# gabrielmittag/NISQA

Measured on AMD Instinct MI355X. Metric: clips/sec (10 s, 48 kHz), higher is better.
Workload: dtype bf16x6 (every GEMM -- CNN, projection, self-attention, pooling: fp32 operands as three exact bf16 terms, 6 MFMA products per term pair, f32 accumulate: all 24 operand mantissa bits; mel f32)

## Files before the change

nisqa_amd/csrc/cnn_bf16.hip:

```cpp
#include "common.hpp"
#include "layout.hpp"
#include <stdlib.h>
#include <atomic>
#include "conv_bf16.hpp"
#include "internal.hpp"
#include "../../include/nisqa_hip.h"
#define NQ_RING2 3
#define NQ_RING34 3

#define FB_RS1 48
#define FB_P1 (168 * FB_RS1)
#define FB_RS2 80
#define FB_P2 (60 * FB_RS2)
#define FB_RS3 144
#define FB_P3 (60 * FB_RS3)
#define FB_PS (72 * FB_RS3)
#define FB_PATCH(T) ((T) * FB_P1)
#define FB_PPLANE 1700
#define FB_ZADDR 2048u
#define FB_BASE 2176u
#define FB_WAVE(T) (((T) * (FB_P1 + FB_PPLANE) + 63u) / 64u * 64u)
#define FB_WGS(T) ((T) == 2 ? 2 : 1)
#define FB_LDS(T) (FB_BASE + 4 * FB_WAVE(T))
static_assert(FB_WAVE(2) == 19584 && FB_LDS(2) == 80512 && 2 * FB_LDS(2) <= 160 * 1024, "two terms: two workgroups (8 waves) per CU");
static_assert(FB_WAVE(3) == 29312 && FB_LDS(3) == 119424 && FB_LDS(3) <= 160 * 1024 && 2 * FB_LDS(3) > 160 * 1024, "three terms: one workgroup per CU");
#define FB_PLAN_OK(T) (FB_PATCH(T) + (T) * FB_PPLANE <= FB_WAVE(T) && (T) * FB_P3 <= FB_WAVE(T) && (T) * FB_PS <= 2 * FB_WAVE(T))
static_assert(FB_PLAN_OK(2) && FB_PLAN_OK(3), "LDS plan");

__device__ constexpr int bwin75_lo(int b) { return b == 0 ? 0 : b == 1 ? 1 : b == 2 ? 2 : b == 3 ? 4 : 5; }
__device__ constexpr int bwin75_hi(int b) { return b == 0 ? 2 : b == 1 ? 3 : b == 2 ? 5 : b == 3 ? 6 : 7; }
__device__ constexpr int bwin53_lo(int b) { return b == 0 ? 0 : b == 1 ? 1 : 3; }
__device__ constexpr int bwin53_hi(int b) { return b == 0 ? 2 : b == 1 ? 4 : 5; }

NQ_CLK_EXPORT(g_phase_clk, nisqa_debug_phase_clock)
NQ_CLK_EXPORT(g_phase_clk6, nisqa_debug_phase_clock6)

#define FB_TAB5 0u
#define FB_TAB6 1024u
NQ_DEV f32x2_t lds_ld64(unsigned a) { return *(NQ_AS3 const f32x2_t*)(a); }
template <int FMT>
NQ_DEV float epi_fmt(float v, float c, float t) {
    return FMT == NQ_FMT_BF16X3 || FMT == NQ_FMT_BF16X6 ? fmaxf(v + t, 0.f) : fmaxf(fmaf(v, c, t), 0.f);
}

template <int FMT, int CIN, int MT, int NT, int W, int RS, int PLANE, bool APF, int RING>
NQ_DEV void fb_conv_k(f32x16 (&acc)[MT][NT], __amdgpu_buffer_rsrc_t wrs, int wbyte, unsigned lane16, const unsigned (&base)[MT],
                      const unsigned (&m9)[MT], conv_k_ring<FMT == NQ_FMT_BF16X6 ? 3 : 2, NT, 3>& ring) {
    if constexpr (FMT == NQ_FMT_BF16X6) conv_k_terms_ring<3, CIN, MT, NT, W, RS, PLANE, FB_ZADDR, 3, true, true>(acc, wrs, wbyte, lane16, base, m9, ring);
    else conv_k_bf16<CIN, MT, NT, W, RS, PLANE, FB_ZADDR, APF, RING, FMT>(acc, wrs, wbyte, lane16, base, m9);
}

template <int FMT, bool SEGX, bool P3>
NQ_DEV void cnn_front_split_body(
    const float* __restrict__ mel_tm, const int32_t* __restrict__ frame_off,
    const int32_t* __restrict__ tok_off, const int32_t* __restrict__ n_wins,
    const float* __restrict__ clip_floor, int n_clips, int seg_hop,
    const float* __restrict__ cw, const unsigned short* __restrict__ wb, float* __restrict__ p3,
    float* __restrict__ feat, const float* __restrict__ seg_x, int seg_L,
    const uint32_t* __restrict__ clip_max_enc, float top_db) {
    extern __shared__ __attribute__((aligned(16))) char smem[];
    constexpr bool X6 = FMT == NQ_FMT_BF16X6, F16 = FMT == NQ_FMT_F16X3 || FMT == NQ_FMT_F16X4;
    constexpr int T = X6 ? 3 : 2;
    static_assert(!P3 || FMT == NQ_FMT_BF16X3, "the fp32 copy of the pooled conv4 tensor is a bf16x3 debug output");
    constexpr int W1_ = X6 ? CNNX_W1 : CNNB_W1, W2_ = X6 ? CNNX_W2 : CNNB_W2, W3_ = X6 ? CNNX_W3 : CNNB_W3, W4_ = X6 ? CNNX_W4 : CNNB_W4,
                  W5_ = X6 ? CNNX_W5 : CNNB_W5, W6_ = X6 ? CNNX_W6 : CNNB_W6, WU16_ = X6 ? CNNX_U16S : CNNB_U16S;
    const int* __restrict__ meta_i = (const int*)(wb + CNNH_META);
    const float* __restrict__ meta_f = (const float*)(wb + CNNH_META);
    float dummy_mx = 0.f;
    NQ_STAMP_BEGIN();
    const int lane = threadIdx.x & 63;
    const int wave = __builtin_amdgcn_readfirstlane(threadIdx.x >> 6);
    const int p0 = blockIdx.x * 4;
    const int b = __builtin_amdgcn_readfirstlane(find_segment_wave(tok_off, n_clips, p0, lane));
    const int k0 = p0 - tok_off[b];
    const int nvalid = min(4, n_wins[b] - k0);
    if (nvalid <= 0) return;
    const bool valid = wave < nvalid;
    const int p = p0 + wave, k = k0 + wave;
    const unsigned R = FB_BASE + wave * FB_WAVE(T);
    const unsigned lane16 = lane * 16;
// ... 10 lines not shown
        vraw[q] = (valid && (q < 11 || lane < 16)) ? src[i0] : 0.f;
    }
    const float tn1 = cw[CNN_T1 + (lane & 15)], tn2 = cw[CNN_T2 + (lane & 31)];
    const float tn3[2] = {cw[CNN_T3 + (lane & 31)], cw[CNN_T3 + 32 + (lane & 31)]};
    const float tn4[2] = {cw[CNN_T4 + (lane & 31)], cw[CNN_T4 + 32 + (lane & 31)]};
    const float tn5 = cw[CNN_T5 + 16 * wave + (lane & 15)], tn6 = cw[CNN_T6 + 16 * wave + (lane & 15)];
    float vin[12];
#pragma unroll
    for (int q = 0; q < 12; ++q) vin[q] = !valid ? 0.f : SEGX ? vraw[q] : fmaxf(vraw[q], fl);
    int e_in = 0;
    float m_in = 0.f;
    float s0 = 1.f;
    if (F16) {
        float mr = 0.f;
#pragma unroll
        for (int q = 0; q < 12; ++q) mr = fmaxf(mr, __builtin_fabsf(vin[q]));
        m_in = wave_max_nonneg(mr);
        e_in = f16_scale_exp(m_in);
        s0 = pow2_f32(e_in);
    }
    {
        const unsigned pb = R + FB_PATCH(T);
        constexpr int NZ = (T * FB_PPLANE + 15) / 16;
#pragma unroll
        for (int it = 0; it < (NZ + 63) / 64; ++it)
            if (64 * it + 64 <= NZ || lane < NZ - 64 * it) lds_st128(pb + (lane + 64 * it) * 16, f32x4{0.f, 0.f, 0.f, 0.f});
        if (lane < 32) ((unsigned*)(smem + FB_ZADDR))[lane] = 0u;
        __builtin_amdgcn_wave_barrier();
        if (!SEGX) {
            unsigned ob[3];
#pragma unroll
            for (int u = 0; u < 3; ++u) {
                const int e = lane + 16 * u, j0 = e >= 48 ? 1 : 0, m = e - 48 * j0;
                ob[u] = pb + ((j0 + 1) * 50 + m + 1) * 2;
            }
#pragma unroll
            for (int q = 0; q < 12; q += 2) {
                const float v0 = vin[q] * s0, v1 = vin[q + 1] * s0;
                lds_store_pair_fmt<FMT>(ob[q % 3] + (q + q / 3) * 100, ob[(q + 1) % 3] + (q + 1 + (q + 1) / 3) * 100, FB_PPLANE, v0, v1,
                                               dummy_mx, true, q + 1 < 11 || lane < 16);
            }
        } else {
#pragma unroll
            for (int q = 0; q < 12; ++q) {
                const int i0 = lane + 64 * q;
                const int m = i0 / 15, j = i0 - 15 * m;
                if (i0 < 720) lds_store_one_fmt<FMT>(pb + ((j + 1) * 50 + (m + 1)) * 2, FB_PPLANE, vin[q] * s0, dummy_mx);
            }
        }
    }
    __builtin_amdgcn_wave_barrier();
    NQ_STAMP(1);

    const int i = lane & 31, hfi = (i >> 2) & 1, qi = (i & 3) + 4 * (i >> 3);
    const int n = lane & 31, hf = lane >> 5, h = lane >> 5;

    conv_k_ring<T, 1, 3> ring2;
    if constexpr (X6) conv_k_preload(ring2, wrs, W2_ * 2, lane16);
    {
        f32x4 w1[1][T];
#pragma unroll
        for (int t = 0; t < T; ++t) w1[0][t] = wfrag_load(wrs, lane16, (W1_ + t * 512) * 2);
        float tn = tn1, c1 = 1.f, ms1 = 0.f;
        int e1 = 0;
        if (F16) {
            e1 = f16_scale_exp(fmaf(m_in, meta_f[8], meta_f[16]));
            c1 = pow2_f32(e1 - e_in - meta_i[0]);
            tn = tn1 * pow2_f32(e1);
        }
        const int xq = min(qi, 14);
        unsigned rd_a = R + FB_PATCH(T) + ((xq + (h ? 2 : 0)) * 50 + 24 * hfi) * 2;
        unsigned rd_b = R + FB_PATCH(T) + ((xq + (h ? 2 : 1)) * 50 + 24 * hfi) * 2;
        const bool is_b = (n & 16) != 0;
        const unsigned mb = is_b ? ~0u : 0u;
        unsigned wr = R + (12 * hf * 7) * FB_RS1 + (n & 15) * 2 + (is_b ? FB_RS1 : 0);
        for (int g2 = 0; g2 < 6; ++g2) {
            f32x16 acc[2][1];
            f32x4 xa[2][T];
#pragma unroll
            for (int tt = 0; tt < 2; ++tt)
#pragma unroll
                for (int t = 0; t < T; ++t) {
                    const unsigned pa = rd_a + 4 * tt + t * FB_PPLANE, pq = rd_b + 4 * tt + t * FB_PPLANE;
                    xa[tt][t] = f32x4{__uint_as_float(lds_ld32(pa)), __uint_as_float(lds_ld32(pa + 4)),
                                      __uint_as_float(lds_ld32(pq)), __uint_as_float(lds_ld32(pq + 4))};
                }
            acc[0][0] = zero16();
            acc[1][0] = zero16();
            if constexpr (X6) {
                mma_terms<T, 2, 1>(acc, xa, w1);
            } else {
                const f32x4 (&w)[T] = w1[0];
                if (FMT == NQ_FMT_F16X4) { acc[0][0] = mfma32_fmt<FMT>(xa[0][1], w[1], acc[0][0]); acc[1][0] = mfma32_fmt<FMT>(xa[1][1], w[1], acc[1][0]); }
                acc[0][0] = mfma32_fmt<FMT>(xa[0][1], w[0], acc[0][0]); acc[1][0] = mfma32_fmt<FMT>(xa[1][1], w[0], acc[1][0]);
                acc[0][0] = mfma32_fmt<FMT>(xa[0][0], w[1], acc[0][0]); acc[1][0] = mfma32_fmt<FMT>(xa[1][0], w[1], acc[1][0]);
                acc[0][0] = mfma32_fmt<FMT>(xa[0][0], w[0], acc[0][0]); acc[1][0] = mfma32_fmt<FMT>(xa[1][0], w[0], acc[1][0]);
            }
            unsigned r[14];
#pragma unroll
            for (int v = 0; v < 14; ++v) {
                const int tt = v / 7, bb = v - 7 * tt;
                const float mx = fmaxf(fmaxf(acc[tt][0][2 * bb], acc[tt][0][2 * bb + 1]), acc[tt][0][2 * bb + 2]);
                r[v] = __float_as_uint(epi_fmt<FMT>(mx, c1, tn));
            }
            unsigned got[7];
#pragma unroll
            for (int kk = 0; kk < 7; ++kk)
                got[kk] = (unsigned)__builtin_amdgcn_ds_swizzle((int)((r[2 * kk] & mb) | (r[2 * kk + 1] & ~mb)), 0x401F);
            float fin[7];
#pragma unroll
            for (int kk = 0; kk < 7; ++kk) {
                const unsigned own = (r[2 * kk + 1] & mb) | (r[2 * kk] & ~mb);
                fin[kk] = __uint_as_float(max(own, got[kk]));
            }
#pragma unroll
            for (int kk = 0; kk < 6; kk += 2) lds_store_pair_fmt<FMT>(wr + 2 * kk * FB_RS1, wr + 2 * (kk + 1) * FB_RS1, FB_P1, fin[kk], fin[kk + 1], ms1);
            lds_store_one_fmt<FMT>(wr + 12 * FB_RS1, FB_P1, fin[6], ms1);
            rd_a += 8; rd_b += 8;
            wr += 14 * FB_RS1;
        }
        if (F16) { m_in = wave_max_nonneg(ms1) * pow2_f32(-e1); e_in = e1; }
    }

    NQ_STAMP(2);
    conv_k_ring<T, 2, 3> ring34;
    {
        f32x16 acc[6][1];
        unsigned base[6], m9[6];
#pragma unroll
        for (int t = 0; t < 6; ++t) {
            acc[t][0] = zero16();
            const int u = 16 * t + qi;
            const int gl = u / 14, w = u % 14, yy = w / 7;
            const int py = 2 * (6 * hfi + gl) + yy, px = w - 7 * yy;
            m9[t] = tap_mask(u < 84, py, px, 24, 7);
            base[t] = R + ((py - 1) * 7 + (px - 1)) * FB_RS1 + (h << 4);
        }
        fb_conv_k<FMT, 16, 6, 1, 7, FB_RS1, FB_P1, false, NQ_RING2>(acc, wrs, W2_ * 2, lane16, base, m9, ring2);
        NQ_STAMP(3);
        if constexpr (X6) {
            conv_k_preload(ring34, wrs, W3_ * 2, lane16);
            __builtin_amdgcn_sched_barrier(0);
        }
        float tn = tn2, c2 = 1.f, ms2 = 0.f;
        int e2 = 0;
        if (F16) {
            e2 = f16_scale_exp(fmaf(m_in, meta_f[9], meta_f[17]));
            c2 = pow2_f32(e2 - e_in - meta_i[1]);
            tn = tn2 * pow2_f32(e2);
        }
        const unsigned wr = R + (6 * hf * 5) * FB_RS2 + n * 2;
#pragma unroll
        for (int k2 = 0; k2 < 30; k2 += 2) {
            float pv[2];
#pragma unroll
            for (int e = 0; e < 2; ++e) {
                const int gl = (k2 + e) / 5, bb = (k2 + e) % 5;
                float mx = -3.0e38f;
#pragma unroll
                for (int yy = 0; yy < 2; ++yy)
#pragma unroll
                    for (int x = bwin75_lo(bb); x < bwin75_hi(bb); ++x) {
                        const int u = 14 * gl + 7 * yy + x;
                        mx = fmaxf(mx, acc[u >> 4][0][u & 15]);
                    }
                pv[e] = epi_fmt<FMT>(mx, c2, tn);
            }
            lds_store_pair_fmt<FMT>(wr + k2 * FB_RS2, wr + (k2 + 1) * FB_RS2, FB_P2, pv[0], pv[1], ms2);
        }
        if (F16) { m_in = wave_max_nonneg(ms2) * pow2_f32(-e2); e_in = e2; }
    }

    NQ_STAMP(4);
    unsigned base34[2], m34[2];
#pragma unroll
    for (int t = 0; t < 2; ++t) {
        const int u = 16 * t + qi;
        const int gl = u / 10, w = u % 10, yy = w / 5;
        const int py = 2 * (3 * hfi + gl) + yy, px = w - 5 * yy;
        m34[t] = tap_mask(u < 30, py, px, 12, 5);
        base34[t] = (py - 1) * 5 + (px - 1);
    }

    {
        f32x16 acc[2][2];
        unsigned base[2];
#pragma unroll
        for (int t = 0; t < 2; ++t) {
#pragma unroll
            for (int nt = 0; nt < 2; ++nt) acc[t][nt] = zero16();
            base[t] = R + base34[t] * FB_RS2 + (h << 4);
        }
        fb_conv_k<FMT, 32, 2, 2, 5, FB_RS2, FB_P2, true, NQ_RING34>(acc, wrs, W3_ * 2, lane16, base, m34, ring34);
        NQ_STAMP(5);
        if constexpr (X6) {
            conv_k_preload(ring34, wrs, W4_ * 2, lane16);
            __builtin_amdgcn_sched_barrier(0);
        }
        float tn[2] = {tn3[0], tn3[1]}, c3 = 1.f, ms3 = 0.f;
        int e3 = 0;
        if (F16) {
            e3 = f16_scale_exp(fmaf(m_in, meta_f[10], meta_f[18]));
            c3 = pow2_f32(e3 - e_in - meta_i[2]);
            tn[0] *= pow2_f32(e3);
            tn[1] *= pow2_f32(e3);
        }
        const unsigned wr = R + (6 * hf * 5) * FB_RS3 + n * 2;
#pragma unroll
        for (int nt = 0; nt < 2; ++nt)
#pragma unroll
            for (int t = 0; t < 2; ++t)
#pragma unroll
                for (int r = 0; r < 16; r += 2) {
                    const int u = 16 * t + r;
                    if (u < 30)
                        lds_store_pair_fmt<FMT>(wr + u * FB_RS3 + 64 * nt, wr + (u + 1) * FB_RS3 + 64 * nt, FB_P3,
                                                epi_fmt<FMT>(acc[t][nt][r], c3, tn[nt]), epi_fmt<FMT>(acc[t][nt][r + 1], c3, tn[nt]), ms3);
                }
        if (F16) { m_in = wave_max_nonneg(ms3) * pow2_f32(-e3); e_in = e3; }
    }

    NQ_STAMP(6);
    const unsigned S4 = FB_BASE;
    const unsigned S5 = FB_BASE + 2 * FB_WAVE(T);
    const int w5b = __builtin_amdgcn_readfirstlane((W5_ + wave * (18 * T * 512)) * 2);
    const int w6b = __builtin_amdgcn_readfirstlane((W6_ + wave * (18 * T * 512)) * 2);
    f32x4 b5[4][T], b6[8][T];
    {
        f32x16 acc[2][2];
        unsigned base[2];
#pragma unroll
        for (int t = 0; t < 2; ++t) {
#pragma unroll
            for (int nt = 0; nt < 2; ++nt) acc[t][nt] = zero16();
            base[t] = R + base34[t] * FB_RS3 + (h << 4);
        }
        fb_conv_k<FMT, 64, 2, 2, 5, FB_RS3, FB_P3, true, NQ_RING34>(acc, wrs, W4_ * 2, lane16, base, m34, ring34);
        NQ_STAMP(7);
        float tn[2] = {tn4[0], tn4[1]}, c4 = 1.f, ms4 = 0.f;
        int e4 = 0;
        if (F16) {
            e4 = f16_scale_exp(fmaf(m_in, meta_f[11], meta_f[19]));
            c4 = pow2_f32(e4 - e_in - meta_i[3]);
            tn[0] *= pow2_f32(e4);
            tn[1] *= pow2_f32(e4);
        }
#pragma unroll
        for (int g = 0; g < 3; ++g)
#pragma unroll
            for (int q = 0; q < T; ++q) b5[g][q] = wfrag_load(wrs, lane16, w5b + (g * T + q) * 1024);
        __syncthreads();
        const unsigned wr = S4 + (18 * wave + 9 * hf) * FB_RS3 + n * 2;
        float* dst = P3 ? p3 + (size_t)p * (18 * 64) : nullptr;
#pragma unroll
        for (int gl = 0; gl < 3; ++gl)
#pragma unroll
            for (int bb = 0; bb < 3; ++bb) {
                float pv[2];
#pragma unroll
                for (int nt = 0; nt < 2; ++nt) {
                    float mx = -3.0e38f;
#pragma unroll
                    for (int yy = 0; yy < 2; ++yy)
#pragma unroll
                        for (int x = bwin53_lo(bb); x < bwin53_hi(bb); ++x) {
                            const int u = 10 * gl + 5 * yy + x;
                            mx = fmaxf(mx, acc[u >> 4][nt][u & 15]);
                        }
                    pv[nt] = epi_fmt<FMT>(mx, c4, tn[nt]);
                    if (P3 && valid) dst[((3 * hf + gl) * 3 + bb) * 64 + n + 32 * nt] = pv[nt];
                }
                lds_store_pair_fmt<FMT>(wr + (gl * 3 + bb) * FB_RS3, wr + (gl * 3 + bb) * FB_RS3 + 64, FB_PS, pv[0], pv[1], ms4);
            }
        if (F16) {
            const float m4 = wave_max_nonneg(ms4) * pow2_f32(-e4);
            const int e5 = f16_scale_exp(fmaf(m4, meta_f[12], meta_f[20]));
            if (lane < 18) {
                lds_st32(FB_TAB5 + (18 * wave + lane) * 8, __float_as_uint(pow2_f32(e5 - e4 - meta_i[4])));
                lds_st32(FB_TAB5 + (18 * wave + lane) * 8 + 4, __float_as_uint(pow2_f32(e5)));
            }
            if (lane < 6) lds_st32(FB_TAB6 + (6 * wave + lane) * 4, __float_as_uint(pow2_f32(-(e5 + meta_i[5]))));
        }
    }
    __syncthreads();
    NQ_STAMP(8);

    {
        const int i16 = lane & 15, kg = lane >> 4;
        const int ch = 16 * wave + i16;
        f32x4 acc5[5];
        unsigned base5[5], m5[5];
#pragma unroll
        for (int t = 0; t < 5; ++t) {
            acc5[t] = f32x4{0.f, 0.f, 0.f, 0.f};
            const int rho = 16 * t + i16;
            const int slot = rho / 18, pix = rho - 18 * slot, ry = pix / 3, rx = pix - 3 * ry;
            m5[t] = tap_mask(rho < 72, ry, rx, 6, 3);
            base5[t] = S4 + (slot * 18 + (ry - 1) * 3 + (rx - 1)) * FB_RS3 + (kg << 4);
        }
        unsigned a5ad[5][T];
        f32x4 a5[2][5][T];
        auto load_a5 = [&](int g) {
            const int tap = g >> 1, s = g & 1;
            const int tapoff = ((tap / 3) * 3 + tap % 3) * FB_RS3;
            if (s == 0) {
#pragma unroll
                for (int t = 0; t < 5; ++t) {
                    const bool ok = (m5[t] >> tap) & 1u;
#pragma unroll
                    for (int q = 0; q < T; ++q) a5ad[t][q] = ok ? base5[t] + q * FB_PS : FB_ZADDR - tapoff;
                }
            }
#pragma unroll
            for (int t = 0; t < 5; ++t)
#pragma unroll
                for (int q = 0; q < T; ++q) a5[g & 1][t][q] = lds_ld128(a5ad[t][q] + tapoff + 64 * s);
        };
        load_a5(0);
#pragma unroll
        for (int g = 0; g < 18; ++g) {
            if (g + 3 < 18) {
#pragma unroll
                for (int q = 0; q < T; ++q) b5[(g + 3) & 3][q] = wfrag_load(wrs, lane16, w5b + ((g + 3) * T + q) * 1024);
            }
            if (g + 1 < 18) load_a5(g + 1);
            if constexpr (X6) {
                __builtin_amdgcn_sched_barrier(0);
                mma16_terms<T, 5>(acc5, a5[g & 1], b5[g & 3]);
            } else mma16_pair_fmt<FMT, 5>(acc5, a5[g & 1], b5[g & 3]);
        }
        NQ_STAMP(9);
#pragma unroll
        for (int g = 0; g < 7; ++g)
#pragma unroll
            for (int q = 0; q < T; ++q) b6[g][q] = wfrag_load(wrs, lane16, w6b + (g * T + q) * 1024);
        {
            const unsigned wr = S5 + (4 * kg) * FB_RS3 + ch * 2;
#pragma unroll
            for (int t = 0; t < 5; ++t)
#pragma unroll
                for (int r = 0; r < 4; r += 2)
                    if (t < 4 || kg < 2) {
                        f32x2_t cs0 = {1.f, 1.f}, cs1 = {1.f, 1.f};
                        if (F16) { cs0 = lds_ld64(FB_TAB5 + (16 * t + r) * 8 + kg * 32); cs1 = lds_ld64(FB_TAB5 + (16 * t + r + 1) * 8 + kg * 32); }
                        lds_store_pair_fmt<FMT>(wr + (16 * t + r) * FB_RS3, wr + (16 * t + r + 1) * FB_RS3, FB_PS,
                                                epi_fmt<FMT>(acc5[t][r], cs0[0], tn5 * cs0[1]), epi_fmt<FMT>(acc5[t][r + 1], cs1[0], tn5 * cs1[1]), dummy_mx);
                    }
        }
        __syncthreads();
        NQ_STAMP(10);

        f32x4 acc6[2], acc6b[2];
        unsigned base6[2], m6[2];
#pragma unroll
        for (int t = 0; t < 2; ++t) {
            acc6[t] = f32x4{0.f, 0.f, 0.f, 0.f};
            acc6b[t] = acc6[t];
            const int rho = 16 * t + i16;
            const int slot = rho / 6, y = rho - 6 * slot;
            m6[t] = tap_mask(rho < 24, y, 1, 6, 3);
            base6[t] = S5 + (slot * 18 + (y - 1) * 3) * FB_RS3 + (kg << 4);
        }
        unsigned a6ad[2][T];
        f32x4 a6[2][2][T];
        auto load_a6 = [&](int g) {
            const int tap = g >> 1, s = g & 1;
            const int tapoff = ((tap / 3) * 3 + tap % 3) * FB_RS3;
            if (s == 0) {
#pragma unroll
                for (int t = 0; t < 2; ++t) {
                    const bool ok = (m6[t] >> tap) & 1u;
#pragma unroll
                    for (int q = 0; q < T; ++q) a6ad[t][q] = ok ? base6[t] + q * FB_PS : FB_ZADDR - tapoff;
                }
            }
#pragma unroll
            for (int t = 0; t < 2; ++t)
#pragma unroll
                for (int q = 0; q < T; ++q) a6[g & 1][t][q] = lds_ld128(a6ad[t][q] + tapoff + 64 * s);
        };
        load_a6(0);
#pragma unroll
        for (int g = 0; g < 18; ++g) {
            if (g + 7 < 18) {
#pragma unroll
                for (int q = 0; q < T; ++q) b6[(g + 7) & 7][q] = wfrag_load(wrs, lane16, w6b + ((g + 7) * T + q) * 1024);
            }
            if (g + 1 < 18) load_a6(g + 1);
            f32x4 (&acc)[2] = (g & 1) ? acc6b : acc6;
            if constexpr (X6) {
                __builtin_amdgcn_sched_barrier(0);
                mma16_terms<T, 2>(acc, a6[g & 1], b6[g & 7]);
            } else mma16_pair_fmt<FMT, 2>(acc, a6[g & 1], b6[g & 7]);
        }
        NQ_STAMP(11);
        const unsigned fo = S4 + wave * 2048;
#pragma unroll
        for (int t = 0; t < 2; ++t)
#pragma unroll
            for (int r = 0; r < 4; ++r) {
                const int rho = 16 * t + 4 * kg + r;
                const int slot = rho / 6, y = rho - 6 * slot;
                if (rho < 24) {
                    const float c6 = F16 ? __uint_as_float(lds_ld32(FB_TAB6 + (16 * t + r) * 4 + kg * 16)) : 1.f;
                    lds_st32(fo + (slot * 96 + i16 * 6 + y) * 4, __float_as_uint(epi_fmt<FMT>(acc6[t][r] + acc6b[t][r], c6, tn6)));
                }
            }
        __builtin_amdgcn_wave_barrier();
#pragma unroll
        for (int q0 = 0; q0 < 96; q0 += 64) {
            const int q = q0 + lane;
            const int slot = q / 24;
            if (q < 96 && slot < nvalid)
                *(f32x4*)(feat + (size_t)(p0 + slot) * 384 + 96 * wave + 4 * (q - 24 * slot)) = lds_ld128(fo + 16 * q);
        }
    }
    NQ_STAMP_END((X6 ? g_phase_clk6 : g_phase_clk), ((blockIdx.y * gridDim.x + blockIdx.x) << 2) + wave);
}

#define FB_PARAMS                                                                                                              \
    const float* __restrict__ mel_tm, const int32_t* __restrict__ frame_off, const int32_t* __restrict__ tok_off,             \
    const int32_t* __restrict__ n_wins, const float* __restrict__ clip_floor, int n_clips, int seg_hop,                       \
    const float* __restrict__ cw, const unsigned short* __restrict__ wb, float* __restrict__ p3, float* __restrict__ feat,    \
    const float* __restrict__ seg_x, int seg_L, const uint32_t* __restrict__ clip_max_enc, float top_db
#define FB_ARGS mel_tm, frame_off, tok_off, n_wins, clip_floor, n_clips, seg_hop, cw, wb, p3, feat, seg_x, seg_L, clip_max_enc, top_db
template <bool SEGX, bool P3>
__global__ __launch_bounds__(256, FB_WGS(2)) void cnn_front_bf16_kernel(FB_PARAMS) {
    cnn_front_split_body<NQ_FMT_BF16X3, SEGX, P3>(FB_ARGS);
}
template <bool P4, bool SEGX>
__global__ __launch_bounds__(256, FB_WGS(2)) void cnn_front_f16_kernel(FB_PARAMS) {
    cnn_front_split_body<P4 ? NQ_FMT_F16X4 : NQ_FMT_F16X3, SEGX, false>(FB_ARGS);
}
template <bool SEGX>
__global__ __launch_bounds__(256, FB_WGS(3)) void cnn_front_bf16x6_kernel(FB_PARAMS) {
    cnn_front_split_body<NQ_FMT_BF16X6, SEGX, false>(FB_ARGS);
}

typedef void (*fb_kernel_t)(const float*, const int32_t*, const int32_t*, const int32_t*, const float*, int, int, const float*,
                            const unsigned short*, float*, float*, const float*, int, const uint32_t*, float);
static int fb_launch(int fmt, bool segx, bool p3, const float* mel_tm, const int32_t* frame_off, const int32_t* tok_off,
                     const int32_t* n_wins, const float* clip_floor, const uint32_t* clip_max_enc, float top_db, int32_t n_clips,
                     int32_t total_tok_padded, int32_t seg_hop, const float* cnn_w, const uint16_t* cnn_wb, float* p3_opt, float* feat,
                     const float* seg_x, int32_t seg_L, void* stream) {
    if (n_clips <= 0 || total_tok_padded <= 0 || (total_tok_padded & 31) || seg_hop <= 0 || !cnn_wb || !feat || fmt < 0 || fmt > 3 ||
        (p3 && fmt != 0) || (segx && (!seg_x || seg_L <= 0)) || (!segx && !clip_floor && !clip_max_enc))
// ... 84 lines not shown
```

nisqa_amd/csrc/conv_bf16.hpp:

```cpp
#pragma once
#include "bf16_terms.hpp"

#define NQ_FMT_BF16X3 0
#define NQ_FMT_F16X3 1
#define NQ_FMT_F16X4 2
#define NQ_FMT_BF16X6 3
typedef _Float16 f16x8 __attribute__((ext_vector_type(8)));
typedef _Float16 f16x2_t __attribute__((ext_vector_type(2)));
template <int FMT>
NQ_DEV f32x16 mfma32_fmt(f32x4 a, f32x4 b, f32x16 c) {
    if (FMT == NQ_FMT_BF16X3) return mfma_bf(a, b, c);
    return __builtin_amdgcn_mfma_f32_32x32x16_f16(__builtin_bit_cast(f16x8, a), __builtin_bit_cast(f16x8, b), c, 0, 0, 0);
}
template <int FMT>
NQ_DEV f32x4 mfma16_fmt(f32x4 a, f32x4 b, f32x4 c) {
    if (FMT == NQ_FMT_BF16X3) return mfma_bf16x16(a, b, c);
    return __builtin_amdgcn_mfma_f32_16x16x32_f16(__builtin_bit_cast(f16x8, a), __builtin_bit_cast(f16x8, b), c, 0, 0, 0);
}
template <int FMT, int MT, int NT>
NQ_DEV void mma_pair_fmt(f32x16 (&acc)[MT][NT], const f32x4 (&ah)[MT], const f32x4 (&al)[MT], const f32x4 (&bh)[NT], const f32x4 (&bl)[NT]) {
    if (FMT == NQ_FMT_F16X4) {
#pragma unroll
        for (int t = 0; t < MT; ++t)
#pragma unroll
            for (int nt = 0; nt < NT; ++nt) acc[t][nt] = mfma32_fmt<FMT>(al[t], bl[nt], acc[t][nt]);
    }
#pragma unroll
    for (int t = 0; t < MT; ++t)
#pragma unroll
        for (int nt = 0; nt < NT; ++nt) acc[t][nt] = mfma32_fmt<FMT>(ah[t], bl[nt], acc[t][nt]);
#pragma unroll
    for (int t = 0; t < MT; ++t)
#pragma unroll
        for (int nt = 0; nt < NT; ++nt) acc[t][nt] = mfma32_fmt<FMT>(al[t], bh[nt], acc[t][nt]);
#pragma unroll
    for (int t = 0; t < MT; ++t)
#pragma unroll
        for (int nt = 0; nt < NT; ++nt) acc[t][nt] = mfma32_fmt<FMT>(ah[t], bh[nt], acc[t][nt]);
}
template <int FMT, int MT>
NQ_DEV void mma16_pair_fmt(f32x4 (&acc)[MT], const f32x4 (&a)[MT][2], const f32x4 (&b)[2]) {
    if (FMT == NQ_FMT_F16X4) {
#pragma unroll
        for (int t = 0; t < MT; ++t) acc[t] = mfma16_fmt<FMT>(a[t][1], b[1], acc[t]);
    }
#pragma unroll
    for (int t = 0; t < MT; ++t) acc[t] = mfma16_fmt<FMT>(a[t][0], b[1], acc[t]);
#pragma unroll
    for (int t = 0; t < MT; ++t) acc[t] = mfma16_fmt<FMT>(a[t][1], b[0], acc[t]);
#pragma unroll
    for (int t = 0; t < MT; ++t) acc[t] = mfma16_fmt<FMT>(a[t][0], b[0], acc[t]);
}
NQ_DEV int f16_scale_exp(float bound) {
    const int be = (int)((__float_as_uint(bound) >> 23) & 0xffu);
// ... 61 lines not shown
    if (FMT == NQ_FMT_BF16X3) { lds_store_split2(a0, a1, plane, v0, v1, st0, st1); return; }
    if (FMT == NQ_FMT_BF16X6) { lds_store_terms2<3>(a0, a1, plane, v0, v1, st0, st1); return; }
    const unsigned hi2 = cvt_pk_f16(v0, v1);
    const f32x2_t vv = {v0, v1};
    const f32x2_t hf = __builtin_convertvector(__builtin_bit_cast(f16x2_t, hi2), f32x2_t);
    const f32x2_t r = vv - hf;
    const unsigned lo2 = cvt_pk_f16(r[0], r[1]);
    mx = fmaxf(fmaxf(mx, __builtin_fabsf(v0)), __builtin_fabsf(v1));
    if (st0) { lds_st16(a0, hi2); lds_st16(a0 + plane, lo2); }
    if (st1) { lds_st16_hi(a1, hi2); lds_st16_hi(a1 + plane, lo2); }
}
template <int FMT>
NQ_DEV void lds_store_one_fmt(unsigned a, int plane, float v, float& mx) {
    if (FMT == NQ_FMT_BF16X3) { lds_store_split(a, plane, v); return; }
    if (FMT == NQ_FMT_BF16X6) { lds_store_terms<3>(a, plane, v); return; }
    const unsigned hi = cvt_pk_f16(v, 0.f);
    const float hf = (float)__builtin_bit_cast(f16x2_t, hi)[0];
    const unsigned lo = cvt_pk_f16(v - hf, 0.f);
    mx = fmaxf(mx, __builtin_fabsf(v));
    lds_st16(a, hi);
    lds_st16(a + plane, lo);
}
NQ_DEV f32x16 splat16(float v) { f32x16 r; for (int q = 0; q < 16; ++q) r[q] = v; return r; }
typedef int nq_i32x4 __attribute__((ext_vector_type(4)));
NQ_DEV f32x4 wfrag_load(__amdgpu_buffer_rsrc_t rsrc, unsigned lane16, int byte_off) {
    return __builtin_bit_cast(f32x4, __builtin_amdgcn_raw_buffer_load_b128(rsrc, lane16, byte_off, 0));
}
NQ_DEV unsigned tap_mask(bool valid, int y, int x, int H, int W) {
    unsigned m = 0;
#pragma unroll
    for (int tap = 0; tap < 9; ++tap) {
        const int yy = y + tap / 3 - 1, xx = x + tap % 3 - 1;
        m |= (valid && (unsigned)yy < (unsigned)H && (unsigned)xx < (unsigned)W) ? (1u << tap) : 0u;
    }
    return m;
}

template <int CIN, int MT, int NT, int W, int RS, int PLANE, unsigned ZADDR, bool APF, int RING = 3, int FMT = NQ_FMT_BF16X3>
NQ_DEV void conv_k_bf16(f32x16 (&acc)[MT][NT], __amdgpu_buffer_rsrc_t rsrc, int wbyte, unsigned lane16,
                        const unsigned (&base)[MT], const unsigned (&m9)[MT]) {
    constexpr int S16 = CIN / 16, TOTAL = 9 * S16, AB = APF ? 2 : 1;
    static_assert(ZADDR >= (2 * W + 2) * RS + 32 * S16, "zero block must sit above the largest tap offset");
    f32x4 bh[RING][NT], bl[RING][NT], ah[AB][MT], al[AB][MT];
    unsigned a_hi[MT], a_lo[MT];
    auto load_b = [&](int g, int slot) {
#pragma unroll
        for (int nt = 0; nt < NT; ++nt) {
            bh[slot][nt] = wfrag_load(rsrc, lane16, wbyte + ((g * NT + nt) * 2 + 0) * 1024);
            bl[slot][nt] = wfrag_load(rsrc, lane16, wbyte + ((g * NT + nt) * 2 + 1) * 1024);
        }
    };
    auto load_a = [&](int g, int slot) {
        const int tap = g / S16, s = g - tap * S16;
        const int tapoff = ((tap / 3) * W + tap % 3) * RS;
        if (s == 0) {
#pragma unroll
            for (int t = 0; t < MT; ++t) {
                const bool ok = (m9[t] >> tap) & 1u;
                a_hi[t] = ok ? base[t] : ZADDR - tapoff;
                a_lo[t] = ok ? base[t] + PLANE : ZADDR - tapoff;
            }
        }
#pragma unroll
        for (int t = 0; t < MT; ++t) {
            ah[slot][t] = lds_ld128(a_hi[t] + tapoff + 32 * s);
            al[slot][t] = lds_ld128(a_lo[t] + tapoff + 32 * s);
        }
    };
#pragma unroll
    for (int g = 0; g < RING - 1; ++g) load_b(g, g);
    if (APF) load_a(0, 0);
#pragma unroll
    for (int g = 0; g < TOTAL; ++g) {
        NQ_STEP_FENCE();
        if (g + RING - 1 < TOTAL) load_b(g + RING - 1, (g + RING - 1) % RING);
        if (APF) { if (g + 1 < TOTAL) load_a(g + 1, (g + 1) & 1); } else load_a(g, 0);
        NQ_ISSUE_FENCE();
        const int sa = APF ? (g & 1) : 0, sb = g % RING;
        mma_pair_fmt<FMT, MT, NT>(acc, ah[sa], al[sa], bh[sb], bl[sb]);
    }
}


template <int T>
NQ_DEV void lds_store_terms2(unsigned a0, unsigned a1, int plane, float v0, float v1, bool st0, bool st1) {
    f32x2_t r = {v0, v1};
#pragma unroll
    for (int t = 0; t < T; ++t) {
        const unsigned pk = cvt_pk_bf16(r[0], r[1]);
        if (st0) lds_st16(a0 + t * plane, pk);
        if (st1) lds_st16_hi(a1 + t * plane, pk);
        if (t + 1 < T) {
            const f32x2_t part = {__uint_as_float(pk << 16), __uint_as_float(pk & 0xffff0000u)};
            r = r - part;
        }
    }
}
template <int T>
NQ_DEV void lds_store_terms(unsigned a, int plane, float v) {
    float r = v;
#pragma unroll
    for (int t = 0; t < T; ++t) {
        const unsigned pk = cvt_pk_bf16(r, 0.f);
        lds_st16(a + t * plane, pk);
        if (t + 1 < T) r -= __uint_as_float(pk << 16);
    }
}
template <int T, int NT, int RING = 3>
struct conv_k_ring { f32x4 b[RING][NT][T]; };
template <int T, int NT, int RING>
NQ_DEV void conv_k_preload(conv_k_ring<T, NT, RING>& r, __amdgpu_buffer_rsrc_t rsrc, int wbyte, unsigned lane16) {
#pragma unroll
    for (int g = 0; g < RING - 1; ++g)
#pragma unroll
        for (int nt = 0; nt < NT; ++nt)
#pragma unroll
            for (int t = 0; t < T; ++t) r.b[g][nt][t] = wfrag_load(rsrc, lane16, wbyte + ((g * NT + nt) * T + t) * 1024);
}
template <int T, int CIN, int MT, int NT, int W, int RS, int PLANE, unsigned ZADDR, int RING, bool FENCE, bool PRE>
NQ_DEV void conv_k_terms_ring(f32x16 (&acc)[MT][NT], __amdgpu_buffer_rsrc_t rsrc, int wbyte, unsigned lane16,
                              const unsigned (&base)[MT], const unsigned (&m9)[MT], conv_k_ring<T, NT, RING>& ring) {
    constexpr int S16 = CIN / 16, TOTAL = 9 * S16;
    static_assert(ZADDR >= (2 * W + 2) * RS + 32 * S16, "zero block must sit above the largest tap offset");
    f32x4 a[2][MT][T];
    unsigned a_ad[MT][T];
    auto load_b = [&](int g, int slot) {
#pragma unroll
        for (int nt = 0; nt < NT; ++nt)
#pragma unroll
            for (int t = 0; t < T; ++t) ring.b[slot][nt][t] = wfrag_load(rsrc, lane16, wbyte + ((g * NT + nt) * T + t) * 1024);
    };
    auto load_a = [&](int g, int slot) {
        const int tap = g / S16, s = g - tap * S16;
        const int tapoff = ((tap / 3) * W + tap % 3) * RS;
        if (s == 0) {
#pragma unroll
            for (int m = 0; m < MT; ++m) {
                const bool ok = (m9[m] >> tap) & 1u;
#pragma unroll
                for (int t = 0; t < T; ++t) a_ad[m][t] = ok ? base[m] + t * PLANE : ZADDR - tapoff;
            }
        }
#pragma unroll
        for (int m = 0; m < MT; ++m)
#pragma unroll
            for (int t = 0; t < T; ++t) a[slot][m][t] = lds_ld128(a_ad[m][t] + tapoff + 32 * s);
    };
    if (!PRE) {
#pragma unroll
        for (int g = 0; g < RING - 1; ++g) load_b(g, g);
    }
    load_a(0, 0);
#pragma unroll
    for (int g = 0; g < TOTAL; ++g) {
        if (g + RING - 1 < TOTAL) load_b(g + RING - 1, (g + RING - 1) % RING);
        if (g + 1 < TOTAL) load_a(g + 1, (g + 1) & 1);
        if (FENCE) __builtin_amdgcn_sched_barrier(0);
        mma_terms<T, MT, NT>(acc, a[g & 1], ring.b[g % RING]);
    }
}
template <int T, int CIN, int MT, int NT, int W, int RS, int PLANE, unsigned ZADDR, int RING = 3, bool FENCE = true>
NQ_DEV void conv_k_terms(f32x16 (&acc)[MT][NT], __amdgpu_buffer_rsrc_t rsrc, int wbyte, unsigned lane16,
                         const unsigned (&base)[MT], const unsigned (&m9)[MT]) {
    conv_k_ring<T, NT, RING> ring;
    conv_k_terms_ring<T, CIN, MT, NT, W, RS, PLANE, ZADDR, RING, FENCE, false>(acc, rsrc, wbyte, lane16, base, m9, ring);
}
```

Measured before the change: 63200.

## Pad conv5/conv6 LDS rows, add per-lane zero window, and triple-buffer A loads

Widens the row stride of the conv4-output and conv5-output staging from 144 to 160 bytes, with compile-time checks that every lane group of the conv5/conv6 A-operand 128-bit LDS reads hits distinct bank slots. Out-of-image taps now read from a zeroed window that keeps each lane's bank offset, instead of one shared zero address. The window is cleared in a new per-wave store. In the six-product path, conv5/conv6 A loads become triple-buffered, and explicit sched_group_barrier sequences interleave the LDS reads, global weight loads and MFMAs. The cost is more registers and somewhat more LDS.

```diff
diff --git a/nisqa_amd/csrc/cnn_bf16.hip b/nisqa_amd/csrc/cnn_bf16.hip
--- a/nisqa_amd/csrc/cnn_bf16.hip
+++ b/nisqa_amd/csrc/cnn_bf16.hip
@@ -3,18 +3,20 @@
 #include <stdlib.h>
 #include <atomic>
 #include "conv_bf16.hpp"
+#include "lds_banks.hpp"
 #include "internal.hpp"
 #include "../../include/nisqa_hip.h"
 #define NQ_RING2 3
 #define NQ_RING34 3
 
-#define FB_RS1 48
+#define FB_RS1 nq_lds::RS_A1
 #define FB_P1 (168 * FB_RS1)
-#define FB_RS2 80
+#define FB_RS2 nq_lds::RS_A2
 #define FB_P2 (60 * FB_RS2)
-#define FB_RS3 144
+#define FB_RS3 nq_lds::RS_A3
 #define FB_P3 (60 * FB_RS3)
-#define FB_PS (72 * FB_RS3)
+#define FB_RSS nq_lds::RS_S
+#define FB_PS (72 * FB_RSS)
 #define FB_PATCH(T) ((T) * FB_P1)
 #define FB_PPLANE 1700
 #define FB_ZADDR 2048u
@@ -26,6 +28,13 @@
 static_assert(FB_WAVE(3) == 29312 && FB_LDS(3) == 119424 && FB_LDS(3) <= 160 * 1024 && 2 * FB_LDS(3) > 160 * 1024, "three terms: one workgroup per CU");
 #define FB_PLAN_OK(T) (FB_PATCH(T) + (T) * FB_PPLANE <= FB_WAVE(T) && (T) * FB_P3 <= FB_WAVE(T) && (T) * FB_PS <= 2 * FB_WAVE(T))
 static_assert(FB_PLAN_OK(2) && FB_PLAN_OK(3), "LDS plan");
+#define FB_ZW(T) ((FB_BASE + (T) * FB_PS + 255u) / 256u * 256u)
+#define FB_ZWN (256 + (2 * 3 + 2) * FB_RSS + 64 + 16)
+static_assert(FB_RSS % 16 == 0 && FB_RSS >= 128 && FB_PS % 256 == 0, "S4 / S5 rows; term planes congruent modulo the bank window");
+static_assert(FB_ZW(2) + 4 * 26 * 16 <= FB_BASE + 2 * FB_WAVE(2) && FB_ZW(3) + 4 * 26 * 16 <= FB_BASE + 2 * FB_WAVE(3), "zero window inside the wave 0 / 1 regions, below S5");
+static_assert(4 * 2048 <= 2 * FB_PS, "the feature staging of conv6's epilogue (2 KB per wave) fits S4");
+static_assert(nq_lds::layer_ways<5>(FB_RSS) == 1 && nq_lds::layer_ways<6>(FB_RSS) == 1,
+              "conv5 / conv6: every lane group of every A-operand ds_read_b128 hits 16 distinct slots, out-of-image taps included");
 
 __device__ constexpr int bwin75_lo(int b) { return b == 0 ? 0 : b == 1 ? 1 : b == 2 ? 2 : b == 3 ? 4 : 5; }
 __device__ constexpr int bwin75_hi(int b) { return b == 0 ? 2 : b == 1 ? 3 : b == 2 ? 5 : b == 3 ? 6 : 7; }
@@ -142,7 +151,7 @@
     __builtin_amdgcn_wave_barrier();
     NQ_STAMP(1);
 
-    const int i = lane & 31, hfi = (i >> 2) & 1, qi = (i & 3) + 4 * (i >> 3);
+    const int hfi = nq_lds::row_hfi(lane), qi = nq_lds::row_qi(lane);
     const int n = lane & 31, hf = lane >> 5, h = lane >> 5;
 
     conv_k_ring<T, 1, 3> ring2;
@@ -220,11 +229,9 @@
 #pragma unroll
         for (int t = 0; t < 6; ++t) {
             acc[t][0] = zero16();
-            const int u = 16 * t + qi;
-            const int gl = u / 14, w = u % 14, yy = w / 7;
-            const int py = 2 * (6 * hfi + gl) + yy, px = w - 7 * yy;
-            m9[t] = tap_mask(u < 84, py, px, 24, 7);
-            base[t] = R + ((py - 1) * 7 + (px - 1)) * FB_RS1 + (h << 4);
+            const nq_lds::pixel px = nq_lds::conv2_pixel(t, qi, hfi);
+            m9[t] = tap_mask(px.valid, px.y, px.x, 24, 7);
+            base[t] = R + nq_lds::a32_base(px, 7, FB_RS1, h);
         }
         fb_conv_k<FMT, 16, 6, 1, 7, FB_RS1, FB_P1, false, NQ_RING2>(acc, wrs, W2_ * 2, lane16, base, m9, ring2);
         NQ_STAMP(3);
@@ -265,11 +272,9 @@
     unsigned base34[2], m34[2];
 #pragma unroll
     for (int t = 0; t < 2; ++t) {
-        const int u = 16 * t + qi;
-        const int gl = u / 10, w = u % 10, yy = w / 5;
-        const int py = 2 * (3 * hfi + gl) + yy, px = w - 5 * yy;
-        m34[t] = tap_mask(u < 30, py, px, 12, 5);
-        base34[t] = (py - 1) * 5 + (px - 1);
+        const nq_lds::pixel px = nq_lds::conv34_pixel(t, qi, hfi);
+        m34[t] = tap_mask(px.valid, px.y, px.x, 12, 5);
+        base34[t] = nq_lds::a32_base(px, 5, 1, 0);
     }
 
     {
@@ -340,7 +345,9 @@
 #pragma unroll
             for (int q = 0; q < T; ++q) b5[g][q] = wfrag_load(wrs, lane16, w5b + (g * T + q) * 1024);
         __syncthreads();
-        const unsigned wr = S4 + (18 * wave + 9 * hf) * FB_RS3 + n * 2;
+        static_assert(4 * 26 * 16 >= FB_ZWN, "zero window: one 16-byte store of 26 lanes per wave");
+        if (lane < 26) lds_st128(FB_ZW(T) + (26 * wave + lane) * 16, f32x4{0.f, 0.f, 0.f, 0.f});
+        const unsigned wr = S4 + (18 * wave + 9 * hf) * FB_RSS + n * 2;
         float* dst = P3 ? p3 + (size_t)p * (18 * 64) : nullptr;
 #pragma unroll
         for (int gl = 0; gl < 3; ++gl)
@@ -360,7 +367,7 @@
                     pv[nt] = epi_fmt<FMT>(mx, c4, tn[nt]);
                     if (P3 && valid) dst[((3 * hf + gl) * 3 + bb) * 64 + n + 32 * nt] = pv[nt];
                 }
-                lds_store_pair_fmt<FMT>(wr + (gl * 3 + bb) * FB_RS3, wr + (gl * 3 + bb) * FB_RS3 + 64, FB_PS, pv[0], pv[1], ms4);
+                lds_store_pair_fmt<FMT>(wr + (gl * 3 + bb) * FB_RSS, wr + (gl * 3 + bb) * FB_RSS + 64, FB_PS, pv[0], pv[1], ms4);
             }
         if (F16) {
             const float m4 = wave_max_nonneg(ms4) * pow2_f32(-e4);
@@ -379,45 +386,55 @@
         const int i16 = lane & 15, kg = lane >> 4;
         const int ch = 16 * wave + i16;
         f32x4 acc5[5];
-        unsigned base5[5], m5[5];
+        unsigned base5[5], zb5[5], m5[5];
 #pragma unroll
         for (int t = 0; t < 5; ++t) {
             acc5[t] = f32x4{0.f, 0.f, 0.f, 0.f};
-            const int rho = 16 * t + i16;
-            const int slot = rho / 18, pix = rho - 18 * slot, ry = pix / 3, rx = pix - 3 * ry;
-            m5[t] = tap_mask(rho < 72, ry, rx, 6, 3);
-            base5[t] = S4 + (slot * 18 + (ry - 1) * 3 + (rx - 1)) * FB_RS3 + (kg << 4);
+            const nq_lds::pixel px = nq_lds::conv5_pixel(t, i16);
+            m5[t] = tap_mask(px.valid, px.y, px.x, 6, 3);
+            base5[t] = S4 + nq_lds::a16_base(nq_lds::conv5_slot(t, i16), px, FB_RSS, kg);
+            zb5[t] = nq_lds::zero_window_base(FB_ZW(T), base5[t]);
         }
         unsigned a5ad[5][T];
-        f32x4 a5[2][5][T];
+        constexpr int AB = X6 ? 3 : 2;
+        f32x4 a5[AB][5][T];
         auto load_a5 = [&](int g) {
             const int tap = g >> 1, s = g & 1;
-            const int tapoff = ((tap / 3) * 3 + tap % 3) * FB_RS3;
+            const int tapoff = nq_lds::tap_offset(tap, 3, FB_RSS);
             if (s == 0) {
 #pragma unroll
                 for (int t = 0; t < 5; ++t) {
                     const bool ok = (m5[t] >> tap) & 1u;
 #pragma unroll
-                    for (int q = 0; q < T; ++q) a5ad[t][q] = ok ? base5[t] + q * FB_PS : FB_ZADDR - tapoff;
+                    for (int q = 0; q < T; ++q) a5ad[t][q] = ok ? base5[t] + q * FB_PS : zb5[t];
                 }
             }
 #pragma unroll
             for (int t = 0; t < 5; ++t)
 #pragma unroll
-                for (int q = 0; q < T; ++q) a5[g & 1][t][q] = lds_ld128(a5ad[t][q] + tapoff + 64 * s);
+                for (int q = 0; q < T; ++q) a5[g % AB][t][q] = lds_ld128(a5ad[t][q] + tapoff + 64 * s);
         };
-        load_a5(0);
+#pragma unroll
+        for (int g = 0; g < AB - 1; ++g) load_a5(g);
 #pragma unroll
         for (int g = 0; g < 18; ++g) {
             if (g + 3 < 18) {
 #pragma unroll
                 for (int q = 0; q < T; ++q) b5[(g + 3) & 3][q] = wfrag_load(wrs, lane16, w5b + ((g + 3) * T + q) * 1024);
             }
-            if (g + 1 < 18) load_a5(g + 1);
+            if (g + AB - 1 < 18) load_a5(g + AB - 1);
             if constexpr (X6) {
+                mma16_terms<T, 5>(acc5, a5[g % AB], b5[g & 3]);
+                if (g + 1 == 18) continue;
+#pragma unroll
+                for (int i = 0; i < 3; ++i) {
+                    __builtin_amdgcn_sched_group_barrier(0x008, 1, 0); __builtin_amdgcn_sched_group_barrier(0x020, 1, 0);
+                    __builtin_amdgcn_sched_group_barrier(0x008, 1, 0); __builtin_amdgcn_sched_group_barrier(0x100, 1, 0);
+                }
+#pragma unroll
+                for (int i = 0; i < 12; ++i) { __builtin_amdgcn_sched_group_barrier(0x008, 2, 0); __builtin_amdgcn_sched_group_barrier(0x100, 1, 0); }
                 __builtin_amdgcn_sched_barrier(0);
-                mma16_terms<T, 5>(acc5, a5[g & 1], b5[g & 3]);
-            } else mma16_pair_fmt<FMT, 5>(acc5, a5[g & 1], b5[g & 3]);
+            } else mma16_pair_fmt<FMT, 5>(acc5, a5[g % AB], b5[g & 3]);
         }
         NQ_STAMP(9);
 #pragma unroll
@@ -425,7 +442,7 @@
 #pragma unroll
             for (int q = 0; q < T; ++q) b6[g][q] = wfrag_load(wrs, lane16, w6b + (g * T + q) * 1024);
         {
-            const unsigned wr = S5 + (4 * kg) * FB_RS3 + ch * 2;
+            const unsigned wr = S5 + (4 * kg) * FB_RSS + ch * 2;
 #pragma unroll
             for (int t = 0; t < 5; ++t)
 #pragma unroll
@@ -433,7 +450,7 @@
                     if (t < 4 || kg < 2) {
                         f32x2_t cs0 = {1.f, 1.f}, cs1 = {1.f, 1.f};
                         if (F16) { cs0 = lds_ld64(FB_TAB5 + (16 * t + r) * 8 + kg * 32); cs1 = lds_ld64(FB_TAB5 + (16 * t + r + 1) * 8 + kg * 32); }
-                        lds_store_pair_fmt<FMT>(wr + (16 * t + r) * FB_RS3, wr + (16 * t + r + 1) * FB_RS3, FB_PS,
+                        lds_store_pair_fmt<FMT>(wr + (16 * t + r) * FB_RSS, wr + (16 * t + r + 1) * FB_RSS, FB_PS,
                                                 epi_fmt<FMT>(acc5[t][r], cs0[0], tn5 * cs0[1]), epi_fmt<FMT>(acc5[t][r + 1], cs1[0], tn5 * cs1[1]), dummy_mx);
                     }
         }
@@ -441,47 +458,56 @@
         NQ_STAMP(10);
 
         f32x4 acc6[2], acc6b[2];
-        unsigned base6[2], m6[2];
+        unsigned base6[2], zb6[2], m6[2];
 #pragma unroll
         for (int t = 0; t < 2; ++t) {
             acc6[t] = f32x4{0.f, 0.f, 0.f, 0.f};
             acc6b[t] = acc6[t];
-            const int rho = 16 * t + i16;
-            const int slot = rho / 6, y = rho - 6 * slot;
-            m6[t] = tap_mask(rho < 24, y, 1, 6, 3);
-            base6[t] = S5 + (slot * 18 + (y - 1) * 3) * FB_RS3 + (kg << 4);
+            const nq_lds::pixel px = nq_lds::conv6_pixel(t, i16);
+            m6[t] = tap_mask(px.valid, px.y, px.x, 6, 3);
+            base6[t] = S5 + nq_lds::a16_base(nq_lds::conv6_slot(t, i16), px, FB_RSS, kg);
+            zb6[t] = nq_lds::zero_window_base(FB_ZW(T), base6[t]);
         }
         unsigned a6ad[2][T];
-        f32x4 a6[2][2][T];
+        f32x4 a6[AB][2][T];
         auto load_a6 = [&](int g) {
             const int tap = g >> 1, s = g & 1;
-            const int tapoff = ((tap / 3) * 3 + tap % 3) * FB_RS3;
+            const int tapoff = nq_lds::tap_offset(tap, 3, FB_RSS);
             if (s == 0) {
 #pragma unroll
                 for (int t = 0; t < 2; ++t) {
                     const bool ok = (m6[t] >> tap) & 1u;
 #pragma unroll
-                    for (int q = 0; q < T; ++q) a6ad[t][q] = ok ? base6[t] + q * FB_PS : FB_ZADDR - tapoff;
+                    for (int q = 0; q < T; ++q) a6ad[t][q] = ok ? base6[t] + q * FB_PS : zb6[t];
                 }
             }
 #pragma unroll
             for (int t = 0; t < 2; ++t)
 #pragma unroll
-                for (int q = 0; q < T; ++q) a6[g & 1][t][q] = lds_ld128(a6ad[t][q] + tapoff + 64 * s);
+                for (int q = 0; q < T; ++q) a6[g % AB][t][q] = lds_ld128(a6ad[t][q] + tapoff + 64 * s);
         };
-        load_a6(0);
+#pragma unroll
+        for (int g = 0; g < AB - 1; ++g) load_a6(g);
 #pragma unroll
         for (int g = 0; g < 18; ++g) {
             if (g + 7 < 18) {
 #pragma unroll
                 for (int q = 0; q < T; ++q) b6[(g + 7) & 7][q] = wfrag_load(wrs, lane16, w6b + ((g + 7) * T + q) * 1024);
             }
-            if (g + 1 < 18) load_a6(g + 1);
+            if (g + AB - 1 < 18) load_a6(g + AB - 1);
             f32x4 (&acc)[2] = (g & 1) ? acc6b : acc6;
             if constexpr (X6) {
+                mma16_terms<T, 2>(acc, a6[g % AB], b6[g & 7]);
+                if (g + 1 == 18) continue;
+#pragma unroll
+                for (int i = 0; i < 3; ++i) {
+                    __builtin_amdgcn_sched_group_barrier(0x008, 1, 0); __builtin_amdgcn_sched_group_barrier(0x020, 1, 0);
+                    __builtin_amdgcn_sched_group_barrier(0x008, 1, 0); __builtin_amdgcn_sched_group_barrier(0x100, 1, 0);
+                }
+#pragma unroll
+                for (int i = 0; i < 3; ++i) { __builtin_amdgcn_sched_group_barrier(0x008, 2, 0); __builtin_amdgcn_sched_group_barrier(0x100, 1, 0); }
                 __builtin_amdgcn_sched_barrier(0);
-                mma16_terms<T, 2>(acc, a6[g & 1], b6[g & 7]);
-            } else mma16_pair_fmt<FMT, 2>(acc, a6[g & 1], b6[g & 7]);
+            } else mma16_pair_fmt<FMT, 2>(acc, a6[g % AB], b6[g & 7]);
         }
         NQ_STAMP(11);
         const unsigned fo = S4 + wave * 2048;
diff --git a/nisqa_amd/csrc/conv_bf16.hpp b/nisqa_amd/csrc/conv_bf16.hpp
--- a/nisqa_amd/csrc/conv_bf16.hpp
+++ b/nisqa_amd/csrc/conv_bf16.hpp
@@ -1,5 +1,6 @@
 #pragma once
 #include "bf16_terms.hpp"
+#include "lds_banks.hpp"
 
 #define NQ_FMT_BF16X3 0
 #define NQ_FMT_F16X3 1
@@ -167,7 +168,7 @@
     };
     auto load_a = [&](int g, int slot) {
         const int tap = g / S16, s = g - tap * S16;
-        const int tapoff = ((tap / 3) * W + tap % 3) * RS;
+        const int tapoff = nq_lds::tap_offset(tap, W, RS);
         if (s == 0) {
 #pragma unroll
             for (int t = 0; t < MT; ++t) {
@@ -247,7 +248,7 @@
     };
     auto load_a = [&](int g, int slot) {
         const int tap = g / S16, s = g - tap * S16;
-        const int tapoff = ((tap / 3) * W + tap % 3) * RS;
+        const int tapoff = nq_lds::tap_offset(tap, W, RS);
         if (s == 0) {
 #pragma unroll
             for (int m = 0; m < MT; ++m) {
diff --git a/nisqa_amd/csrc/lds_banks.hpp b/nisqa_amd/csrc/lds_banks.hpp
--- /dev/null
+++ b/nisqa_amd/csrc/lds_banks.hpp
@@ -0,0 +1,125 @@
+#pragma once
+
+#if defined(__HIPCC__) || defined(__CUDACC__)
+#define NQ_LDS_HD __host__ __device__
+#else
+#define NQ_LDS_HD
+#endif
+
+namespace nq_lds {
+
+NQ_LDS_HD constexpr int b128_group(int lane) {
+    const int l = lane & 31;
+    const bool first = l < 4 || (l >= 12 && l < 16) || (l >= 20 && l < 28);
+    return 2 * (lane >> 5) + (first ? 0 : 1);
+}
+NQ_LDS_HD constexpr int b128_slot(int byte_addr) { return (byte_addr >> 4) & 15; }
+template <class F>
+NQ_LDS_HD constexpr int b128_ways(const F& addr) {
+    int worst = 0;
+    for (int g = 0; g < 4; ++g) {
+        int seen[16][16] = {}, n[16] = {};
+        for (int lane = 0; lane < 64; ++lane) {
+            if (b128_group(lane) != g) continue;
+            const int a = addr(lane);
+            if (a < 0) continue;
+            const int s = b128_slot(a);
+            bool dup = false;
+            for (int k = 0; k < n[s]; ++k) dup = dup || seen[s][k] == a;
+            if (!dup) seen[s][n[s]++] = a;
+            if (n[s] > worst) worst = n[s];
+        }
+    }
+    return worst;
+}
+template <class F>
+NQ_LDS_HD constexpr unsigned b128_slot_set(const F& addr, int g) {
+    unsigned m = 0;
+    for (int lane = 0; lane < 64; ++lane)
+        if (b128_group(lane) == g && addr(lane) >= 0) m |= 1u << b128_slot(addr(lane));
+    return m;
+}
+template <class F>
+NQ_LDS_HD constexpr int b128_lanes(const F& addr, int g) {
+    int n = 0;
+    for (int lane = 0; lane < 64; ++lane) n += (b128_group(lane) == g && addr(lane) >= 0) ? 1 : 0;
+    return n;
+}
+
+constexpr int RS_A1 = 48;
+constexpr int RS_A2 = 80;
+constexpr int RS_A3 = 144;
+constexpr int RS_S = 160;
+
+struct pixel { int y, x; bool valid; };
+NQ_LDS_HD constexpr bool tap_inside(pixel p, int tap, int H, int W) {
+    const int yy = p.y + tap / 3 - 1, xx = p.x + tap % 3 - 1;
+    return p.valid && yy >= 0 && yy < H && xx >= 0 && xx < W;
+}
+NQ_LDS_HD constexpr int tap_offset(int tap, int W, int rs) { return ((tap / 3) * W + tap % 3) * rs; }
+
+NQ_LDS_HD constexpr int row_hfi(int lane) { return (lane >> 2) & 1; }
+NQ_LDS_HD constexpr int row_qi(int lane) { return (lane & 3) + 4 * ((lane & 31) >> 3); }
+NQ_LDS_HD constexpr pixel conv2_pixel(int t, int qi, int hfi) {
+    const int u = 16 * t + qi, gl = u / 14, w = u % 14, yy = w / 7;
+    return pixel{2 * (6 * hfi + gl) + yy, w - 7 * yy, u < 84};
+}
+NQ_LDS_HD constexpr pixel conv34_pixel(int t, int qi, int hfi) {
+    const int u = 16 * t + qi, gl = u / 10, w = u % 10, yy = w / 5;
+    return pixel{2 * (3 * hfi + gl) + yy, w - 5 * yy, u < 30};
+}
+NQ_LDS_HD constexpr int a32_base(pixel p, int W, int rs, int h) { return ((p.y - 1) * W + (p.x - 1)) * rs + (h << 4); }
+template <int LAYER>
+struct a32_read {
+    int rs, t, tap;
+    NQ_LDS_HD constexpr int operator()(int lane) const {
+        const pixel p = LAYER == 2 ? conv2_pixel(t, row_qi(lane), row_hfi(lane)) : conv34_pixel(t, row_qi(lane), row_hfi(lane));
+        const int H = LAYER == 2 ? 24 : 12, W = LAYER == 2 ? 7 : 5;
+        if (!tap_inside(p, tap, H, W)) return -1;
+        return 65536 + a32_base(p, W, rs, lane >> 5) + tap_offset(tap, W, rs);
+    }
+};
+
+NQ_LDS_HD constexpr int conv5_slot(int t, int i16) { return (16 * t + i16) / 18; }
+NQ_LDS_HD constexpr pixel conv5_pixel(int t, int i16) {
+    const int rho = 16 * t + i16, pix = rho % 18;
+    return pixel{pix / 3, pix % 3, rho < 72};
+}
+NQ_LDS_HD constexpr int conv6_slot(int t, int i16) { return (16 * t + i16) / 6; }
+NQ_LDS_HD constexpr pixel conv6_pixel(int t, int i16) {
+    const int rho = 16 * t + i16;
+    return pixel{rho % 6, 1, rho < 24};
+}
+NQ_LDS_HD constexpr int a16_base(int slot, pixel p, int rs, int kg) { return (slot * 18 + (p.y - 1) * 3 + (p.x - 1)) * rs + (kg << 4); }
+NQ_LDS_HD constexpr unsigned zero_window_base(unsigned zw, unsigned base) { return zw + (base & 255u); }
+template <int LAYER>
+struct a16_read {
+    int rs, t, tap;
+    bool window = true;
+    int plane = 65536 + 128, zw = 1 << 20;
+    NQ_LDS_HD constexpr int operator()(int lane) const {
+        const int i16 = lane & 15, kg = lane >> 4;
+        const pixel p = LAYER == 5 ? conv5_pixel(t, i16) : conv6_pixel(t, i16);
+        const int slot = LAYER == 5 ? conv5_slot(t, i16) : conv6_slot(t, i16);
+        const int base = plane + a16_base(slot, p, rs, kg);
+        if (tap_inside(p, tap, 6, 3)) return base + tap_offset(tap, 3, rs);
+        return window ? (int)zero_window_base((unsigned)zw, (unsigned)base) + tap_offset(tap, 3, rs) : -1;
+    }
+};
+
+template <int LAYER>
+NQ_LDS_HD constexpr int layer_tiles() { return LAYER == 2 ? 6 : LAYER == 5 ? 5 : 2; }
+template <int LAYER>
+NQ_LDS_HD constexpr int layer_ways(int rs, bool window = true) {
+    int worst = 0;
+    for (int t = 0; t < layer_tiles<LAYER>(); ++t)
+        for (int tap = 0; tap < 9; ++tap) {
+            int w = 0;
+            if constexpr (LAYER >= 5) w = b128_ways(a16_read<LAYER>{rs, t, tap, window});
+            else w = b128_ways(a32_read<LAYER>{rs, t, tap});
+            if (w > worst) worst = w;
+        }
+    return worst;
+}
+
+}
```

Result: no change. 63360 (median of 3 runs) (+0.2%).
